# Aleph-Alpha/magma

Measured on NVIDIA H100. Metric: image-caption samples/sec (fwd+bwd), higher is better.
Workload: dtype bf16

## Files before the change

### magma_b200/csrc/attention.cu

```cuda
#include <stdlib.h>

#include "gemm_common.cuh"

namespace mb200 {

static constexpr int kAttThreads = 256;
static constexpr int kTile = 128 * 64 * 2;

struct AttnParams {
  int S, H, hd, rot;
  float scale;
  bf16* P;
  long long ldP;
  bf16* O;
  long long ldo;
  bf16* dqkv;
  long long ld_dqkv;
  const float2* rope_tab;
};

__device__ __forceinline__ void fence_async_smem() { asm volatile("fence.proxy.async.shared::cta;" ::: "memory"); }
__device__ __forceinline__ void wg_sync(int wg) { asm volatile("bar.sync %0, 128;" ::"r"(wg + 1) : "memory"); }

__device__ __forceinline__ uint32_t operand_off(int r, int c) {
  return (uint32_t)((c >> 6) * kTile + r * 128 + ((((c & 63) >> 3) ^ (r & 7)) << 4) + (c & 7) * 2);
}
__device__ __forceinline__ void st_pair(uint32_t saddr, float a, float b) {
  asm volatile("st.shared.b32 [%0], %1;" ::"r"(saddr), "r"(f32x2_to_bf16(a, b)) : "memory");
}
__device__ __forceinline__ float2 ld_pair(uint32_t saddr) {
  uint32_t u;
  asm volatile("ld.shared.b32 %0, [%1];" : "=r"(u) : "r"(saddr));
  return bf16x2_to_f32(u);
}
__device__ __forceinline__ float quad_max(float v) {
  v = fmaxf(v, __shfl_xor_sync(0xffffffffu, v, 1));
  return fmaxf(v, __shfl_xor_sync(0xffffffffu, v, 2));
}
__device__ __forceinline__ float quad_sum(float v) {
  v += __shfl_xor_sync(0xffffffffu, v, 1);
  return v + __shfl_xor_sync(0xffffffffu, v, 2);
}

template <int N, bool A_MN, bool B_MN>
__device__ __forceinline__ void wg_mma(float (&d)[N / 2], int wg, uint32_t a_base, uint32_t b_base, int nkb,
                                       uint32_t acc0 = 0u) {
  a_base += A_MN ? (uint32_t)(wg * kTile) : (uint32_t)(wg * 64 * 128);
  wgmma_fence();
  for (int kb = 0; kb < nkb; ++kb) {
#pragma unroll
    for (int k = 0; k < 4; ++k) {
      const uint32_t ao = A_MN ? (uint32_t)((kb * 4 + k) * 2048) : (uint32_t)(kb * kTile + k * 32);
      const uint32_t bo = B_MN ? (uint32_t)((kb * 4 + k) * 2048) : (uint32_t)(kb * kTile + k * 32);
      const uint64_t da = make_smem_desc(a_base + ao, A_MN ? (uint32_t)kTile : 0u, 1024);
      const uint64_t db = make_smem_desc(b_base + bo, B_MN ? (uint32_t)kTile : 0u, 1024);
      wgmma_bf16<N, A_MN ? 1 : 0, B_MN ? 1 : 0>(d, da, db, ((kb | k) != 0 ? 1u : 0u) | acc0);
    }
  }
  wgmma_commit();
  wgmma_wait<0>();
}

struct Frag {
  int wg, r0, c0, quad0;
  __device__ __forceinline__ Frag() {
    const int t = threadIdx.x;
    wg = t >> 7;
    r0 = wg * 64 + ((t & 127) >> 5) * 16 + ((t & 31) >> 2);
    c0 = 2 * (t & 3);
    quad0 = (t & 3) == 0;
  }
};

template <int HD>
__device__ __forceinline__ void store_rows(const Frag& f, const float (&d)[HD / 2], bf16* dst, long long ld, int nrows,
                                           const float2* tab, int rot) {
#pragma unroll
  for (int h = 0; h < 2; ++h) {
    const int r = f.r0 + 8 * h;
    if (r >= nrows) continue;
    bf16* row = dst + (long long)r * ld;
#pragma unroll
    for (int j = 0; j < HD / 8; ++j) {
      const int c = 8 * j + f.c0;
      float a0 = d[4 * j + 2 * h], a1 = d[4 * j + 2 * h + 1];
      if (tab != nullptr && c < rot) {
        const float2 cs = __ldg(tab + (long long)r * (rot >> 1) + (c >> 1));
        const float b0 = a0 * cs.x + a1 * cs.y;
        a1 = a1 * cs.x - a0 * cs.y;
        a0 = b0;
      }
      *reinterpret_cast<uint32_t*>(row + c) = f32x2_to_bf16(a0, a1);
    }
  }
}

template <int HD>
__global__ void __launch_bounds__(kAttThreads, 1)
attn_fwd_tile_kernel(const __grid_constant__ CUtensorMap tmQ, const __grid_constant__ CUtensorMap tmK,
                     const __grid_constant__ CUtensorMap tmV, const AttnParams p) {
  extern __shared__ uint8_t smem_raw[];
  uint8_t* smem = reinterpret_cast<uint8_t*>((reinterpret_cast<uintptr_t>(smem_raw) + 1023) & ~uintptr_t(1023));
  constexpr int nhb = HD / 64;
  uint8_t* sQ = smem;
  uint8_t* sK = sQ + nhb * kTile;
  uint8_t* sV = sK + nhb * kTile;
  uint8_t* sP = sV + nhb * kTile;
  uint64_t* bars = reinterpret_cast<uint64_t*>(sP + 2 * kTile);
  uint64_t* bar_qk = bars + 0;
  uint64_t* bar_v = bars + 1;

  const int t = threadIdx.x;
  const int h = blockIdx.x % p.H, b = blockIdx.x / p.H;
  const Frag f;

  pdl_trigger();
  if (t == 0) {
    tma_prefetch_desc(&tmQ);
    tma_prefetch_desc(&tmK);
    tma_prefetch_desc(&tmV);
    for (int i = 0; i < 2; ++i) mbar_init(&bars[i], 1);
    mbar_fence_init();
  }
  __syncthreads();
  pdl_wait();

  if (t == 0) {
    mbar_expect_tx(bar_qk, 2 * nhb * kTile);
    for (int kb = 0; kb < nhb; ++kb) {
      tma_load_4d(sQ + kb * kTile, &tmQ, bar_qk, kb * 64, 0, h, b);
      tma_load_4d(sK + kb * kTile, &tmK, bar_qk, kb * 64, 0, h, b);
    }
    mbar_expect_tx(bar_v, nhb * kTile);
    for (int kb = 0; kb < nhb; ++kb) tma_load_4d(sV + kb * kTile, &tmV, bar_v, kb * 64, 0, h, b);
  }
  mbar_wait(bar_qk, 0);
  float s[64];
  wg_mma<128, false, false>(s, f.wg, smem_u32(sQ), smem_u32(sK), nhb);
  const uint32_t sP_s = smem_u32(sP);
#pragma unroll
  for (int hh = 0; hh < 2; ++hh) {
    const int q = f.r0 + 8 * hh;
    const int lim = min(p.S, q + 1);
    float m = -INFINITY;
#pragma unroll
    for (int j = 0; j < 16; ++j)
#pragma unroll
      for (int e = 0; e < 2; ++e) {
        float& v = s[4 * j + 2 * hh + e];
        v *= p.scale;
        if (8 * j + f.c0 + e < lim) m = fmaxf(m, v);
      }
    m = quad_max(m);
    float sum = 0.f;
#pragma unroll
    for (int j = 0; j < 16; ++j)
#pragma unroll
      for (int e = 0; e < 2; ++e) {
        float& v = s[4 * j + 2 * hh + e];
        v = 8 * j + f.c0 + e < lim ? __expf(v - m) : 0.f;
        sum += v;
      }
    sum = quad_sum(sum);
    const float inv = q < p.S ? 1.f / sum : 0.f;
    bf16* prow = p.P + (((long long)b * p.H + h) * p.S + q) * p.ldP;
#pragma unroll
    for (int j = 0; j < 16; ++j) {
      const int c = 8 * j + f.c0;
      const float a0 = s[4 * j + 2 * hh] * inv, a1 = s[4 * j + 2 * hh + 1] * inv;
      st_pair(sP_s + operand_off(q, c), a0, a1);
      if (q < p.S && c < p.ldP) *reinterpret_cast<uint32_t*>(prow + c) = f32x2_to_bf16(a0, a1);
    }
  }
  fence_async_smem();
  wg_sync(f.wg);
  mbar_wait(bar_v, 0);
  float o[HD / 2];
  wg_mma<HD, false, true>(o, f.wg, sP_s, smem_u32(sV), 2);
// ... 121 lines not shown
  uint64_t* bars = reinterpret_cast<uint64_t*>(sP + 2 * kTile);
  uint64_t* bar_q = bars + 0;
  uint64_t* bar_k = bars + 1;
  uint64_t* bar_v = bars + 3;

  const int t = threadIdx.x;
  const int q0 = blockIdx.x * 128, h = blockIdx.y, b = blockIdx.z;
  const Frag f;

  pdl_trigger();
  if (t == 0) {
    tma_prefetch_desc(&tmQ);
    tma_prefetch_desc(&tmK);
    tma_prefetch_desc(&tmV);
    for (int i = 0; i < 5; ++i) mbar_init(&bars[i], 1);
    mbar_fence_init();
  }
  __syncthreads();
  pdl_wait();

  int n_kv = (p.Sk + 127) >> 7;
  if (p.causal) {
    const int last_key = min(p.Sk - 1, q0 + 127 + p.kv_off);
    n_kv = last_key < 0 ? 0 : min(n_kv, (last_key >> 7) + 1);
  }
  int row_lim[2];
  bool row_ok[2];
#pragma unroll
  for (int hh = 0; hh < 2; ++hh) {
    const int qi = q0 + f.r0 + 8 * hh;
    row_lim[hh] = !p.causal ? p.Sk : min(p.Sk, qi + p.kv_off + 1);
    row_ok[hh] = qi < p.Sq;
  }

  uint32_t ph_k[2] = {0, 0}, ph_v[2] = {0, 0};
  auto load_k = [&](int j, int buf) {
    mbar_expect_tx(&bar_k[buf], nhb * kTile);
    for (int kb = 0; kb < nhb; ++kb) tma_load_4d(sK + (buf * nhb + kb) * kTile, &tmK, &bar_k[buf], kb * 64, j * 128, h, b);
  };
  auto load_v = [&](int j, int buf) {
    mbar_expect_tx(&bar_v[buf], nhb * kTile);
    for (int kb = 0; kb < nhb; ++kb) tma_load_4d(sV + (buf * nhb + kb) * kTile, &tmV, &bar_v[buf], kb * 64, j * 128, h, b);
  };

  float m[2] = {-INFINITY, -INFINITY}, l[2] = {0.f, 0.f};
  if (t == 0 && n_kv > 0) {
    mbar_expect_tx(bar_q, nhb * kTile);
    for (int kb = 0; kb < nhb; ++kb) tma_load_4d(sQ + kb * kTile, &tmQ, bar_q, kb * 64, q0, h, b);
    load_k(0, 0);
  }
  if (n_kv > 0) mbar_wait(bar_q, 0);
  float s[64];
  for (int j = 0; j < n_kv; ++j) {
    const int buf = NBUF == 2 ? (j & 1) : 0;
    if (t == 0) {
      if (NBUF == 2 && j + 1 < n_kv) load_k(j + 1, (j + 1) & 1);
      if (NBUF == 1 && j + 1 < n_kv)
        for (int kb = 0; kb < nhb; ++kb) tma_prefetch_4d(&tmK, kb * 64, (j + 1) * 128, h, b);
    }
    mbar_wait(&bar_k[buf], ph_k[buf]);
    ph_k[buf] ^= 1;
    wg_mma<128, false, false>(s, f.wg, smem_u32(sQ), smem_u32(sK + buf * nhb * kTile), nhb);
    __syncthreads();
    if (NBUF == 1 && t == 0 && j + 1 < n_kv) load_k(j + 1, 0);
    const int kbase = j * 128;
#pragma unroll
    for (int hh = 0; hh < 2; ++hh) {
      float cm = -INFINITY;
#pragma unroll
      for (int jj = 0; jj < 16; ++jj)
#pragma unroll
        for (int e = 0; e < 2; ++e)
          if (kbase + 8 * jj + f.c0 + e < row_lim[hh]) cm = fmaxf(cm, s[4 * jj + 2 * hh + e] * p.scale);
      cm = quad_max(cm);
      if (cm > m[hh]) {
        l[hh] *= __expf(m[hh] - cm);
        m[hh] = cm;
      }
      if (m[hh] != -INFINITY) {
        float ls = 0.f;
#pragma unroll
        for (int jj = 0; jj < 16; ++jj)
#pragma unroll
          for (int e = 0; e < 2; ++e)
            if (kbase + 8 * jj + f.c0 + e < row_lim[hh]) ls += __expf(s[4 * jj + 2 * hh + e] * p.scale - m[hh]);
        l[hh] += quad_sum(ls);
      }
    }
  }
  float inv[2];
#pragma unroll
  for (int hh = 0; hh < 2; ++hh) {
    inv[hh] = (row_ok[hh] && l[hh] > 0.f) ? 1.f / l[hh] : 0.f;
    if (m[hh] == -INFINITY) m[hh] = 0.f;
    if (p.stats != nullptr && row_ok[hh] && f.quad0)
      p.stats[((long long)b * p.H + h) * p.Sq + q0 + f.r0 + 8 * hh] = make_float2(m[hh], inv[hh]);
  }

  const uint32_t sP_s = smem_u32(sP);
  if (t == 0 && n_kv > 0) {
    load_k(0, 0);
    load_v(0, 0);
  }
  float o[HD / 2];
#pragma unroll
  for (int i = 0; i < HD / 2; ++i) o[i] = 0.f;
  for (int j = 0; j < n_kv; ++j) {
    const int buf = NBUF == 2 ? (j & 1) : 0;
    if (t == 0) {
      if (NBUF == 2 && j + 1 < n_kv) {
        load_k(j + 1, (j + 1) & 1);
        load_v(j + 1, (j + 1) & 1);
      }
      if (NBUF == 1 && j + 1 < n_kv)
        for (int kb = 0; kb < nhb; ++kb) {
          tma_prefetch_4d(&tmK, kb * 64, (j + 1) * 128, h, b);
          tma_prefetch_4d(&tmV, kb * 64, (j + 1) * 128, h, b);
        }
    }
    mbar_wait(&bar_k[buf], ph_k[buf]);
    ph_k[buf] ^= 1;
    wg_mma<128, false, false>(s, f.wg, smem_u32(sQ), smem_u32(sK + buf * nhb * kTile), nhb);
    __syncthreads();
    if (NBUF == 1 && t == 0 && j + 1 < n_kv) load_k(j + 1, 0);
    const int kbase = j * 128;
#pragma unroll
    for (int hh = 0; hh < 2; ++hh) {
      const int r = f.r0 + 8 * hh;
      bf16* prow = p.P ? p.P + (((long long)b * p.H + h) * p.Sq + q0 + r) * p.ldP : nullptr;
#pragma unroll
      for (int jj = 0; jj < 16; ++jj) {
        const int c = 8 * jj + f.c0;
        float a[2];
#pragma unroll
        for (int e = 0; e < 2; ++e)
          a[e] = kbase + c + e < row_lim[hh] ? __expf(s[4 * jj + 2 * hh + e] * p.scale - m[hh]) * inv[hh] : 0.f;
        st_pair(sP_s + operand_off(r, c), a[0], a[1]);
        if (prow != nullptr && row_ok[hh] && kbase + c < p.ldP)
          *reinterpret_cast<uint32_t*>(prow + kbase + c) = f32x2_to_bf16(a[0], a[1]);
      }
    }
    fence_async_smem();
    wg_sync(f.wg);
    mbar_wait(&bar_v[buf], ph_v[buf]);
    ph_v[buf] ^= 1;
    wg_mma<HD, false, true>(o, f.wg, sP_s, smem_u32(sV + buf * nhb * kTile), 2, 1u);
    __syncthreads();
    if (NBUF == 1 && t == 0 && j + 1 < n_kv) load_v(j + 1, 0);
  }
  store_rows<HD>(f, o, p.O + ((long long)b * p.Sq + q0) * p.ldo + (long long)h * HD, p.ldo, p.Sq - q0, nullptr, 0);
  if (p.P != nullptr && t < 128 && q0 + t < p.Sq) {
    bf16* prow = p.P + (((long long)b * p.H + h) * p.Sq + q0 + t) * p.ldP;
    for (int col = n_kv * 128; col < p.ldP; col += 8) *reinterpret_cast<uint4*>(prow + col) = make_uint4(0, 0, 0, 0);
  }
}

static int tile_map(CUtensorMap* m, const void* ptr, long long ld, long long bs0, long long bs1, int rows, int cols,
                    int H, int B) {
  mb200_operand op;
  op.ptr = ptr;
  op.ld = ld;
  op.bs0 = bs0;
  op.bs1 = bs1;
  op.mn_major = 0;
  op.static_data = 0;
  return make_operand_map(m, op, rows, cols, H, B, 128);
}

static constexpr int smem_max = 232448;

bool attn_tile_supported(int S, int hd) { return S >= 1 && S <= 128 && hd >= 64 && hd <= 256 && hd % 64 == 0; }

int attn_fwd_tile(const bf16* qkv, long long ld_qkv, bf16* P, long long ldP, bf16* O, long long ldo, int B, int S, int H,
                  int hd, cudaStream_t st) {
  MB_REQUIRE(attn_tile_supported(S, hd) && ldP % 8 == 0, MB200_E_SHAPE, "attn_fwd_tile: unsupported S=%d hd=%d", S, hd);
  CUtensorMap tq, tk, tv;
  const long long d = (long long)H * hd;
  int rc;
  if ((rc = tile_map(&tq, qkv, ld_qkv, hd, (long long)S * ld_qkv, S, hd, H, B))) return rc;
  if ((rc = tile_map(&tk, qkv + d, ld_qkv, hd, (long long)S * ld_qkv, S, hd, H, B))) return rc;
  if ((rc = tile_map(&tv, qkv + 2 * d, ld_qkv, hd, (long long)S * ld_qkv, S, hd, H, B))) return rc;
  AttnParams p;
  memset(&p, 0, sizeof(p));
  p.S = S;
  p.H = H;
  p.hd = hd;
  p.scale = 1.0f / sqrtf((float)hd);
  p.P = P;
  p.ldP = ldP;
  p.O = O;
  p.ldo = ldo;
  const int smem = (3 * (hd / 64) + 2) * kTile + 1024 + 128;
#define MB_FWD(HD)                                                                                                   \
  {                                                                                                                  \
    static bool set = false;                                                                                         \
    if (!set) {                                                                                                      \
      MB_CUDA(cudaFuncSetAttribute(attn_fwd_tile_kernel<HD>, cudaFuncAttributeMaxDynamicSharedMemorySize, smem_max)); \
      set = true;                                                                                                    \
    }                                                                                                                \
    MB_CUDA(launch_pdl(attn_fwd_tile_kernel<HD>, dim3(B * H), dim3(kAttThreads), (size_t)smem, st, tq, tk, tv, p));  \
  }
  switch (hd) {
    case 64: MB_FWD(64) break;
    case 128: MB_FWD(128) break;
    case 192: MB_FWD(192) break;
    default: MB_FWD(256) break;
  }
#undef MB_FWD
  count_launch();
  return 0;
}

int attn_bwd_tile(const bf16* qkv, long long ld_qkv, const bf16* dO, long long ld_do, const bf16* P, long long ldP,
                  bf16* dqkv, long long ld_dqkv, const float* rope_tab, int rot, int B, int S, int H, int hd,
                  cudaStream_t st) {
  MB_REQUIRE(attn_tile_supported(S, hd) && ldP % 8 == 0, MB200_E_SHAPE, "attn_bwd_tile: unsupported S=%d hd=%d", S, hd);
  CUtensorMap tq, tk, tv, tdo, tp;
  const long long d = (long long)H * hd;
  int rc;
  if ((rc = tile_map(&tq, qkv, ld_qkv, hd, (long long)S * ld_qkv, S, hd, H, B))) return rc;
  if ((rc = tile_map(&tk, qkv + d, ld_qkv, hd, (long long)S * ld_qkv, S, hd, H, B))) return rc;
  if ((rc = tile_map(&tv, qkv + 2 * d, ld_qkv, hd, (long long)S * ld_qkv, S, hd, H, B))) return rc;
  if ((rc = tile_map(&tdo, dO, ld_do, hd, (long long)S * ld_do, S, hd, H, B))) return rc;
  if ((rc = tile_map(&tp, P, ldP, (long long)S * ldP, (long long)H * S * ldP, S, S, H, B))) return rc;
  AttnParams p;
  memset(&p, 0, sizeof(p));
  p.S = S;
  p.H = H;
  p.hd = hd;
  p.rot = rot;
  p.scale = 1.0f / sqrtf((float)hd);
  p.P = const_cast<bf16*>(P);
  p.ldP = ldP;
  p.dqkv = dqkv;
  p.ld_dqkv = ld_dqkv;
  p.rope_tab = reinterpret_cast<const float2*>(rope_tab);
  const int smem = (2 * (hd / 64) + 4) * kTile + 1024 + 128;
#define MB_BWD(HD)                                                                                                   \
  {                                                                                                                  \
    static bool set = false;                                                                                         \
    if (!set) {                                                                                                      \
      MB_CUDA(cudaFuncSetAttribute(attn_bwd_tile_kernel<HD>, cudaFuncAttributeMaxDynamicSharedMemorySize, smem_max)); \
      set = true;                                                                                                    \
    }                                                                                                                \
    MB_CUDA(launch_pdl(attn_bwd_tile_kernel<HD>, dim3(B * H), dim3(kAttThreads), (size_t)smem, st, tq, tk, tv, tdo,  \
                       tp, p));                                                                                      \
  }
  switch (hd) {
    case 64: MB_BWD(64) break;
    case 128: MB_BWD(128) break;
    case 192: MB_BWD(192) break;
    default: MB_BWD(256) break;
  }
#undef MB_BWD
  count_launch();
  return 0;
}

bool attn_flash_supported(int hd) { return hd >= 64 && hd <= 256 && hd % 64 == 0; }

int attn_fwd_flash(const bf16* q, long long ldq, long long q_bsh, long long q_bsb, const bf16* k, long long ldk,
                   long long k_bsh, long long k_bsb, const bf16* v, long long ldv, long long v_bsh, long long v_bsb,
                   bf16* O, long long ldo, bf16* P, long long ldP, float* stats, int B, int Sq, int Sk, int H, int hd,
                   int causal, cudaStream_t st) {
  MB_REQUIRE(attn_flash_supported(hd) && Sq >= 1 && Sk >= 1 && B >= 1 && H >= 1, MB200_E_SHAPE,
             "attn_fwd_flash: unsupported Sq=%d Sk=%d hd=%d", Sq, Sk, hd);
  MB_REQUIRE(!causal || Sk >= Sq, MB200_E_SHAPE, "attn_fwd_flash: causal needs Sk >= Sq (%d < %d)", Sk, Sq);
  MB_REQUIRE(P == nullptr || (ldP % 8 == 0 && ldP >= Sk), MB200_E_ALIGN, "attn_fwd_flash: ldP=%lld must be >= Sk and %%8",
             ldP);
  MB_REQUIRE(ldo % 8 == 0 && (reinterpret_cast<uintptr_t>(O) & 15) == 0, MB200_E_ALIGN, "attn_fwd_flash: O alignment");
  CUtensorMap tq, tk, tv;
  int rc;
  if ((rc = tile_map(&tq, q, ldq, q_bsh, q_bsb, Sq, hd, H, B))) return rc;
  if ((rc = tile_map(&tk, k, ldk, k_bsh, k_bsb, Sk, hd, H, B))) return rc;
  if ((rc = tile_map(&tv, v, ldv, v_bsh, v_bsb, Sk, hd, H, B))) return rc;
  FlashParams p;
  memset(&p, 0, sizeof(p));
  p.Sq = Sq;
  p.Sk = Sk;
  p.H = H;
  p.hd = hd;
  p.causal = causal;
  p.kv_off = Sk - Sq;
  p.scale = 1.0f / sqrtf((float)hd);
  p.O = O;
  p.ldo = ldo;
  p.P = P;
  p.ldP = ldP;
  p.stats = reinterpret_cast<float2*>(stats);
  const dim3 grid((Sq + 127) / 128, H, B);
#define MB_FLASH(HD, NB)                                                                                             \
  {                                                                                                                  \
    const int smem = ((1 + 2 * NB) * (HD / 64) + 2) * kTile + 1024 + 128;                                           \
    static bool set = false;                                                                                         \
    if (!set) {                                                                                                      \
      MB_CUDA(cudaFuncSetAttribute(attn_fwd_flash_kernel<HD, NB>, cudaFuncAttributeMaxDynamicSharedMemorySize,      \
                                   smem_max));                                                                       \
      set = true;                                                                                                    \
    }                                                                                                                \
    MB_CUDA(launch_pdl(attn_fwd_flash_kernel<HD, NB>, grid, dim3(kAttThreads), (size_t)smem, st, tq, tk, tv, p));    \
  }
  switch (hd) {
    case 64: MB_FLASH(64, 2) break;
    case 128: MB_FLASH(128, 2) break;
    case 192: MB_FLASH(192, 1) break;
    default: MB_FLASH(256, 1) break;
  }
#undef MB_FLASH
  count_launch();
  return 0;
}

}

extern "C" int mb200_attn_fwd_tile(const void* qkv, int64_t ld_qkv, void* P, int64_t ldP, void* O, int64_t ldo, int32_t B,
                                   int32_t S, int32_t H, int32_t hd, void* stream) {
  int rc = mb200::check_arch();
  if (rc) return rc;
  return mb200::attn_fwd_tile((const mb200::bf16*)qkv, ld_qkv, (mb200::bf16*)P, ldP, (mb200::bf16*)O, ldo, B, S, H, hd,
                              (cudaStream_t)stream);
}

extern "C" int mb200_attn_bwd_tile(const void* qkv, int64_t ld_qkv, const void* dO, int64_t ld_do, const void* P,
                                   int64_t ldP, void* dqkv, int64_t ld_dqkv, const float* rope_tab, int32_t rot,
                                   int32_t B, int32_t S, int32_t H, int32_t hd, void* stream) {
  int rc = mb200::check_arch();
  if (rc) return rc;
  return mb200::attn_bwd_tile((const mb200::bf16*)qkv, ld_qkv, (const mb200::bf16*)dO, ld_do, (const mb200::bf16*)P, ldP,
                              (mb200::bf16*)dqkv, ld_dqkv, rope_tab, rot, B, S, H, hd, (cudaStream_t)stream);
}

extern "C" int mb200_attn_fwd_flash(const void* q, int64_t ldq, int64_t q_bsh, int64_t q_bsb, const void* k, int64_t ldk,
                                    int64_t k_bsh, int64_t k_bsb, const void* v, int64_t ldv, int64_t v_bsh, int64_t v_bsb,
                                    void* O, int64_t ldo, void* P, int64_t ldP, float* stats, int32_t B, int32_t Sq,
                                    int32_t Sk, int32_t H, int32_t hd, int32_t causal, void* stream) {
  int rc = mb200::check_arch();
  if (rc) return rc;
  return mb200::attn_fwd_flash((const mb200::bf16*)q, ldq, q_bsh, q_bsb, (const mb200::bf16*)k, ldk, k_bsh, k_bsb,
                               (const mb200::bf16*)v, ldv, v_bsh, v_bsb, (mb200::bf16*)O, ldo, (mb200::bf16*)P, ldP, stats,
                               B, Sq, Sk, H, hd, causal, (cudaStream_t)stream);
}
```

### magma_b200/csrc/wgmma.cuh

```cuda

__device__ __forceinline__ void wgmma_fence() { asm volatile("wgmma.fence.sync.aligned;" ::: "memory"); }
__device__ __forceinline__ void wgmma_commit() { asm volatile("wgmma.commit_group.sync.aligned;" ::: "memory"); }
template <int N>
__device__ __forceinline__ void wgmma_wait() { asm volatile("wgmma.wait_group.sync.aligned %0;" ::"n"(N) : "memory"); }

__device__ __forceinline__ uint64_t make_smem_desc(uint32_t saddr, uint32_t lbo_bytes, uint32_t sbo_bytes) {
  uint64_t d = 0;
  d |= (uint64_t)((saddr >> 4) & 0x3FFF);
  d |= (uint64_t)((lbo_bytes >> 4) & 0x3FFF) << 16;
  d |= (uint64_t)((sbo_bytes >> 4) & 0x3FFF) << 32;
  d |= (uint64_t)1 << 62;
  return d;
}

template <int TA, int TB>
__device__ __forceinline__ void wgmma_bf16_n64(float (&d)[32], uint64_t da, uint64_t db, uint32_t accumulate) {
  asm volatile(
      "{\n\t"
      ".reg .pred p;\n\t"
      "setp.ne.b32 p, %34, 0;\n\t"
      "wgmma.mma_async.sync.aligned.m64n64k16.f32.bf16.bf16 "
      "{%0, %1, %2, %3, %4, %5, %6, %7, %8, %9, %10, %11, %12, %13, %14, %15, %16, %17, %18, %19, %20, %21, %22, %23, %24, %25, %26, %27, %28, %29, %30, %31}, "
      "%32, %33, p, 1, 1, %35, %36;\n\t"
      "}\n"
      : "+f"(d[0]), "+f"(d[1]), "+f"(d[2]), "+f"(d[3]), "+f"(d[4]), "+f"(d[5]), "+f"(d[6]), "+f"(d[7]), "+f"(d[8]), "+f"(d[9]), "+f"(d[10]), "+f"(d[11]), "+f"(d[12]), "+f"(d[13]), "+f"(d[14]), "+f"(d[15]), "+f"(d[16]), "+f"(d[17]), "+f"(d[18]), "+f"(d[19]), "+f"(d[20]), "+f"(d[21]), "+f"(d[22]), "+f"(d[23]), "+f"(d[24]), "+f"(d[25]), "+f"(d[26]), "+f"(d[27]), "+f"(d[28]), "+f"(d[29]), "+f"(d[30]), "+f"(d[31])
      : "l"(da), "l"(db), "r"(accumulate), "n"(TA), "n"(TB));
}

template <int TA, int TB>
__device__ __forceinline__ void wgmma_bf16_n128(float (&d)[64], uint64_t da, uint64_t db, uint32_t accumulate) {
  asm volatile(
      "{\n\t"
      ".reg .pred p;\n\t"
      "setp.ne.b32 p, %66, 0;\n\t"
      "wgmma.mma_async.sync.aligned.m64n128k16.f32.bf16.bf16 "
      "{%0, %1, %2, %3, %4, %5, %6, %7, %8, %9, %10, %11, %12, %13, %14, %15, %16, %17, %18, %19, %20, %21, %22, %23, %24, %25, %26, %27, %28, %29, %30, %31, %32, %33, %34, %35, %36, %37, %38, %39, %40, %41, %42, %43, %44, %45, %46, %47, %48, %49, %50, %51, %52, %53, %54, %55, %56, %57, %58, %59, %60, %61, %62, %63}, "
      "%64, %65, p, 1, 1, %67, %68;\n\t"
      "}\n"
      : "+f"(d[0]), "+f"(d[1]), "+f"(d[2]), "+f"(d[3]), "+f"(d[4]), "+f"(d[5]), "+f"(d[6]), "+f"(d[7]), "+f"(d[8]), "+f"(d[9]), "+f"(d[10]), "+f"(d[11]), "+f"(d[12]), "+f"(d[13]), "+f"(d[14]), "+f"(d[15]), "+f"(d[16]), "+f"(d[17]), "+f"(d[18]), "+f"(d[19]), "+f"(d[20]), "+f"(d[21]), "+f"(d[22]), "+f"(d[23]), "+f"(d[24]), "+f"(d[25]), "+f"(d[26]), "+f"(d[27]), "+f"(d[28]), "+f"(d[29]), "+f"(d[30]), "+f"(d[31]), "+f"(d[32]), "+f"(d[33]), "+f"(d[34]), "+f"(d[35]), "+f"(d[36]), "+f"(d[37]), "+f"(d[38]), "+f"(d[39]), "+f"(d[40]), "+f"(d[41]), "+f"(d[42]), "+f"(d[43]), "+f"(d[44]), "+f"(d[45]), "+f"(d[46]), "+f"(d[47]), "+f"(d[48]), "+f"(d[49]), "+f"(d[50]), "+f"(d[51]), "+f"(d[52]), "+f"(d[53]), "+f"(d[54]), "+f"(d[55]), "+f"(d[56]), "+f"(d[57]), "+f"(d[58]), "+f"(d[59]), "+f"(d[60]), "+f"(d[61]), "+f"(d[62]), "+f"(d[63])
      : "l"(da), "l"(db), "r"(accumulate), "n"(TA), "n"(TB));
}

template <int TA, int TB>
__device__ __forceinline__ void wgmma_bf16_n192(float (&d)[96], uint64_t da, uint64_t db, uint32_t accumulate) {
  asm volatile(
      "{\n\t"
      ".reg .pred p;\n\t"
      "setp.ne.b32 p, %98, 0;\n\t"
      "wgmma.mma_async.sync.aligned.m64n192k16.f32.bf16.bf16 "
      "{%0, %1, %2, %3, %4, %5, %6, %7, %8, %9, %10, %11, %12, %13, %14, %15, %16, %17, %18, %19, %20, %21, %22, %23, %24, %25, %26, %27, %28, %29, %30, %31, %32, %33, %34, %35, %36, %37, %38, %39, %40, %41, %42, %43, %44, %45, %46, %47, %48, %49, %50, %51, %52, %53, %54, %55, %56, %57, %58, %59, %60, %61, %62, %63, %64, %65, %66, %67, %68, %69, %70, %71, %72, %73, %74, %75, %76, %77, %78, %79, %80, %81, %82, %83, %84, %85, %86, %87, %88, %89, %90, %91, %92, %93, %94, %95}, "
      "%96, %97, p, 1, 1, %99, %100;\n\t"
      "}\n"
      : "+f"(d[0]), "+f"(d[1]), "+f"(d[2]), "+f"(d[3]), "+f"(d[4]), "+f"(d[5]), "+f"(d[6]), "+f"(d[7]), "+f"(d[8]), "+f"(d[9]), "+f"(d[10]), "+f"(d[11]), "+f"(d[12]), "+f"(d[13]), "+f"(d[14]), "+f"(d[15]), "+f"(d[16]), "+f"(d[17]), "+f"(d[18]), "+f"(d[19]), "+f"(d[20]), "+f"(d[21]), "+f"(d[22]), "+f"(d[23]), "+f"(d[24]), "+f"(d[25]), "+f"(d[26]), "+f"(d[27]), "+f"(d[28]), "+f"(d[29]), "+f"(d[30]), "+f"(d[31]), "+f"(d[32]), "+f"(d[33]), "+f"(d[34]), "+f"(d[35]), "+f"(d[36]), "+f"(d[37]), "+f"(d[38]), "+f"(d[39]), "+f"(d[40]), "+f"(d[41]), "+f"(d[42]), "+f"(d[43]), "+f"(d[44]), "+f"(d[45]), "+f"(d[46]), "+f"(d[47]), "+f"(d[48]), "+f"(d[49]), "+f"(d[50]), "+f"(d[51]), "+f"(d[52]), "+f"(d[53]), "+f"(d[54]), "+f"(d[55]), "+f"(d[56]), "+f"(d[57]), "+f"(d[58]), "+f"(d[59]), "+f"(d[60]), "+f"(d[61]), "+f"(d[62]), "+f"(d[63]), "+f"(d[64]), "+f"(d[65]), "+f"(d[66]), "+f"(d[67]), "+f"(d[68]), "+f"(d[69]), "+f"(d[70]), "+f"(d[71]), "+f"(d[72]), "+f"(d[73]), "+f"(d[74]), "+f"(d[75]), "+f"(d[76]), "+f"(d[77]), "+f"(d[78]), "+f"(d[79]), "+f"(d[80]), "+f"(d[81]), "+f"(d[82]), "+f"(d[83]), "+f"(d[84]), "+f"(d[85]), "+f"(d[86]), "+f"(d[87]), "+f"(d[88]), "+f"(d[89]), "+f"(d[90]), "+f"(d[91]), "+f"(d[92]), "+f"(d[93]), "+f"(d[94]), "+f"(d[95])
      : "l"(da), "l"(db), "r"(accumulate), "n"(TA), "n"(TB));
}

template <int TA, int TB>
__device__ __forceinline__ void wgmma_bf16_n256(float (&d)[128], uint64_t da, uint64_t db, uint32_t accumulate) {
  asm volatile(
      "{\n\t"
      ".reg .pred p;\n\t"
      "setp.ne.b32 p, %130, 0;\n\t"
      "wgmma.mma_async.sync.aligned.m64n256k16.f32.bf16.bf16 "
      "{%0, %1, %2, %3, %4, %5, %6, %7, %8, %9, %10, %11, %12, %13, %14, %15, %16, %17, %18, %19, %20, %21, %22, %23, %24, %25, %26, %27, %28, %29, %30, %31, %32, %33, %34, %35, %36, %37, %38, %39, %40, %41, %42, %43, %44, %45, %46, %47, %48, %49, %50, %51, %52, %53, %54, %55, %56, %57, %58, %59, %60, %61, %62, %63, %64, %65, %66, %67, %68, %69, %70, %71, %72, %73, %74, %75, %76, %77, %78, %79, %80, %81, %82, %83, %84, %85, %86, %87, %88, %89, %90, %91, %92, %93, %94, %95, %96, %97, %98, %99, %100, %101, %102, %103, %104, %105, %106, %107, %108, %109, %110, %111, %112, %113, %114, %115, %116, %117, %118, %119, %120, %121, %122, %123, %124, %125, %126, %127}, "
      "%128, %129, p, 1, 1, %131, %132;\n\t"
      "}\n"
      : "+f"(d[0]), "+f"(d[1]), "+f"(d[2]), "+f"(d[3]), "+f"(d[4]), "+f"(d[5]), "+f"(d[6]), "+f"(d[7]), "+f"(d[8]), "+f"(d[9]), "+f"(d[10]), "+f"(d[11]), "+f"(d[12]), "+f"(d[13]), "+f"(d[14]), "+f"(d[15]), "+f"(d[16]), "+f"(d[17]), "+f"(d[18]), "+f"(d[19]), "+f"(d[20]), "+f"(d[21]), "+f"(d[22]), "+f"(d[23]), "+f"(d[24]), "+f"(d[25]), "+f"(d[26]), "+f"(d[27]), "+f"(d[28]), "+f"(d[29]), "+f"(d[30]), "+f"(d[31]), "+f"(d[32]), "+f"(d[33]), "+f"(d[34]), "+f"(d[35]), "+f"(d[36]), "+f"(d[37]), "+f"(d[38]), "+f"(d[39]), "+f"(d[40]), "+f"(d[41]), "+f"(d[42]), "+f"(d[43]), "+f"(d[44]), "+f"(d[45]), "+f"(d[46]), "+f"(d[47]), "+f"(d[48]), "+f"(d[49]), "+f"(d[50]), "+f"(d[51]), "+f"(d[52]), "+f"(d[53]), "+f"(d[54]), "+f"(d[55]), "+f"(d[56]), "+f"(d[57]), "+f"(d[58]), "+f"(d[59]), "+f"(d[60]), "+f"(d[61]), "+f"(d[62]), "+f"(d[63]), "+f"(d[64]), "+f"(d[65]), "+f"(d[66]), "+f"(d[67]), "+f"(d[68]), "+f"(d[69]), "+f"(d[70]), "+f"(d[71]), "+f"(d[72]), "+f"(d[73]), "+f"(d[74]), "+f"(d[75]), "+f"(d[76]), "+f"(d[77]), "+f"(d[78]), "+f"(d[79]), "+f"(d[80]), "+f"(d[81]), "+f"(d[82]), "+f"(d[83]), "+f"(d[84]), "+f"(d[85]), "+f"(d[86]), "+f"(d[87]), "+f"(d[88]), "+f"(d[89]), "+f"(d[90]), "+f"(d[91]), "+f"(d[92]), "+f"(d[93]), "+f"(d[94]), "+f"(d[95]), "+f"(d[96]), "+f"(d[97]), "+f"(d[98]), "+f"(d[99]), "+f"(d[100]), "+f"(d[101]), "+f"(d[102]), "+f"(d[103]), "+f"(d[104]), "+f"(d[105]), "+f"(d[106]), "+f"(d[107]), "+f"(d[108]), "+f"(d[109]), "+f"(d[110]), "+f"(d[111]), "+f"(d[112]), "+f"(d[113]), "+f"(d[114]), "+f"(d[115]), "+f"(d[116]), "+f"(d[117]), "+f"(d[118]), "+f"(d[119]), "+f"(d[120]), "+f"(d[121]), "+f"(d[122]), "+f"(d[123]), "+f"(d[124]), "+f"(d[125]), "+f"(d[126]), "+f"(d[127])
      : "l"(da), "l"(db), "r"(accumulate), "n"(TA), "n"(TB));
}

template <int N, int TA, int TB>
__device__ __forceinline__ void wgmma_bf16(float (&d)[N / 2], uint64_t da, uint64_t db, uint32_t accumulate) {
  static_assert(N == 64 || N == 128 || N == 192 || N == 256, "wgmma_bf16: N must be 64, 128, 192 or 256");
  if constexpr (N == 64) wgmma_bf16_n64<TA, TB>(d, da, db, accumulate);
  else if constexpr (N == 128) wgmma_bf16_n128<TA, TB>(d, da, db, accumulate);
  else if constexpr (N == 192) wgmma_bf16_n192<TA, TB>(d, da, db, accumulate);
  else wgmma_bf16_n256<TA, TB>(d, da, db, accumulate);
}
```

Measured before the change: 158.8.

## Add specialized short-key flash attention forward kernel for head dim 64

Adds a dedicated forward attention kernel for non-causal hd=64 with up to 272 keys. It loads all of K and V once per block in 64-row TMA boxes, computes scores with one m64n256 plus one m64n16 wgmma per k-step, and does the whole softmax in one pass with no online rescaling across KV tiles. Each CTA handles up to five 64-row query slabs split across two warpgroups, which cuts per-tile loop overhead and barriers. The cost is a large register footprint (128+8 score floats per thread) and a hard-coded key limit.

```diff
diff --git a/magma_b200/csrc/attention.cu b/magma_b200/csrc/attention.cu
--- a/magma_b200/csrc/attention.cu
+++ b/magma_b200/csrc/attention.cu
@@ -22,8 +22,8 @@
 __device__ __forceinline__ void fence_async_smem() { asm volatile("fence.proxy.async.shared::cta;" ::: "memory"); }
 __device__ __forceinline__ void wg_sync(int wg) { asm volatile("bar.sync %0, 128;" ::"r"(wg + 1) : "memory"); }
 
-__device__ __forceinline__ uint32_t operand_off(int r, int c) {
-  return (uint32_t)((c >> 6) * kTile + r * 128 + ((((c & 63) >> 3) ^ (r & 7)) << 4) + (c & 7) * 2);
+__device__ __forceinline__ uint32_t operand_off(int r, int c, uint32_t kb_bytes = kTile) {
+  return (uint32_t)((c >> 6) * kb_bytes + r * 128 + ((((c & 63) >> 3) ^ (r & 7)) << 4) + (c & 7) * 2);
 }
 __device__ __forceinline__ void st_pair(uint32_t saddr, float a, float b) {
   asm volatile("st.shared.b32 [%0], %1;" ::"r"(saddr), "r"(f32x2_to_bf16(a, b)) : "memory");
@@ -454,8 +454,152 @@
   }
 }
 
+static constexpr int kShortKeys = 272;
+static constexpr int kShortBlocks = 5;
+static constexpr int kBox64 = 64 * 64 * 2;
+
+__global__ void __launch_bounds__(kAttThreads, 1)
+attn_fwd_shortkey_kernel(const __grid_constant__ CUtensorMap tmQ, const __grid_constant__ CUtensorMap tmK,
+                         const __grid_constant__ CUtensorMap tmV, const FlashParams p) {
+  extern __shared__ uint8_t smem_raw[];
+  uint8_t* smem = reinterpret_cast<uint8_t*>((reinterpret_cast<uintptr_t>(smem_raw) + 1023) & ~uintptr_t(1023));
+  uint8_t* sQ = smem;
+  uint8_t* sK = sQ + kShortBlocks * kBox64;
+  uint8_t* sV = sK + kShortBlocks * kBox64;
+  uint8_t* sP = sV + kShortBlocks * kBox64;
+  uint64_t* bars = reinterpret_cast<uint64_t*>(sP + 2 * kShortBlocks * kBox64);
+  uint64_t* bar_qk = bars + 0;
+  uint64_t* bar_v = bars + 1;
+
+  const int t = threadIdx.x;
+  const int q0 = blockIdx.x * kShortBlocks * 64, h = blockIdx.y, b = blockIdx.z;
+  const int nslab = min(kShortBlocks, (p.Sq - q0 + 63) >> 6);
+  const int nkb = (p.Sk + 63) >> 6;
+  const Frag f;
+  const int lr0 = f.r0 & 63;
+
+  pdl_trigger();
+  if (t == 0) {
+    tma_prefetch_desc(&tmQ);
+    tma_prefetch_desc(&tmK);
+    tma_prefetch_desc(&tmV);
+    for (int i = 0; i < 2; ++i) mbar_init(&bars[i], 1);
+    mbar_fence_init();
+  }
+  for (int kb = nkb; kb < kShortBlocks; ++kb) {
+    for (int i = t; i < kBox64 / 16; i += kAttThreads) {
+      reinterpret_cast<uint4*>(sK + kb * kBox64)[i] = make_uint4(0, 0, 0, 0);
+      reinterpret_cast<uint4*>(sV + kb * kBox64)[i] = make_uint4(0, 0, 0, 0);
+    }
+  }
+  fence_async_smem();
+  __syncthreads();
+  pdl_wait();
+
+  if (t == 0) {
+    mbar_expect_tx(bar_qk, (nslab + nkb) * kBox64);
+    for (int s = 0; s < nslab; ++s) tma_load_4d(sQ + s * kBox64, &tmQ, bar_qk, 0, q0 + s * 64, h, b);
+    for (int kb = 0; kb < nkb; ++kb) tma_load_4d(sK + kb * kBox64, &tmK, bar_qk, 0, kb * 64, h, b);
+    mbar_expect_tx(bar_v, nkb * kBox64);
+    for (int kb = 0; kb < nkb; ++kb) tma_load_4d(sV + kb * kBox64, &tmV, bar_v, 0, kb * 64, h, b);
+  }
+  const uint32_t sP_s = smem_u32(sP) + (uint32_t)(f.wg * kShortBlocks * kBox64);
+  const uint32_t sK_s = smem_u32(sK), sV_s = smem_u32(sV);
+  mbar_wait(bar_qk, 0);
+  bool v_ready = false;
+  for (int slab = f.wg; slab < nslab; slab += 2) {
+    const int qs = q0 + slab * 64;
+    float s0[128], s1[8];
+    {
+      const uint32_t a = smem_u32(sQ) + (uint32_t)(slab * kBox64);
+      wgmma_fence();
+#pragma unroll
+      for (int k = 0; k < 4; ++k) {
+        const uint64_t da = make_smem_desc(a + k * 32, 0u, 1024);
+        wgmma_bf16<256, 0, 0>(s0, da, make_smem_desc(sK_s + k * 32, 0u, 1024), k != 0 ? 1u : 0u);
+        wgmma_bf16<16, 0, 0>(s1, da, make_smem_desc(sK_s + 4 * kBox64 + k * 32, 0u, 1024), k != 0 ? 1u : 0u);
+      }
+      wgmma_commit();
+      wgmma_wait<0>();
+    }
+#pragma unroll
+    for (int hh = 0; hh < 2; ++hh) {
+      const int lr = lr0 + 8 * hh, q = qs + lr;
+      const bool row_ok = q < p.Sq;
+      float m = -INFINITY, l = 0.f;
+#pragma unroll
+      for (int ch = 0; ch < 3; ++ch) {
+        const int j0 = ch < 2 ? 16 * ch : 0, nj = ch < 2 ? 16 : 2;
+        float* sc = ch < 2 ? s0 : s1;
+        float cm = -INFINITY;
+#pragma unroll
+        for (int jj = 0; jj < nj; ++jj)
+#pragma unroll
+          for (int e = 0; e < 2; ++e)
+            cm = fmaxf(cm, 128 * ch + 8 * jj + f.c0 + e < p.Sk ? sc[4 * (j0 + jj) + 2 * hh + e] * p.scale : -INFINITY);
+        cm = quad_max(cm);
+        if (cm > m) {
+          l *= __expf(m - cm);
+          m = cm;
+        }
+        if (m != -INFINITY) {
+          float ls = 0.f;
+#pragma unroll
+          for (int jj = 0; jj < nj; ++jj)
+#pragma unroll
+            for (int e = 0; e < 2; ++e)
+              ls += 128 * ch + 8 * jj + f.c0 + e < p.Sk ? __expf(sc[4 * (j0 + jj) + 2 * hh + e] * p.scale - m) : 0.f;
+          l += quad_sum(ls);
+        }
+      }
+      const float inv = 1.f / l;
+      if (p.stats != nullptr && row_ok && f.quad0)
+        p.stats[((long long)b * p.H + h) * p.Sq + q] = make_float2(m, inv);
+      bf16* prow = p.P != nullptr && row_ok ? p.P + (((long long)b * p.H + h) * p.Sq + q) * p.ldP : nullptr;
+#pragma unroll
+      for (int j = 0; j < kShortBlocks * 8; ++j) {
+        const int c = 8 * j + f.c0;
+        float a[2];
+#pragma unroll
+        for (int e = 0; e < 2; ++e) {
+          const float sv = j < 32 ? s0[4 * j + 2 * hh + e] : j < 34 ? s1[4 * (j - 32) + 2 * hh + e] : 0.f;
+          a[e] = c + e < p.Sk ? __expf(sv * p.scale - m) * inv : 0.f;
+        }
+        const float a0 = a[0], a1 = a[1];
+        st_pair(sP_s + operand_off(lr, c, kBox64), a0, a1);
+        if (prow != nullptr && c < p.ldP) *reinterpret_cast<uint32_t*>(prow + c) = f32x2_to_bf16(a0, a1);
+      }
+      if (prow != nullptr)
+        for (int c = 64 * kShortBlocks + f.c0; c < p.ldP; c += 8) *reinterpret_cast<uint32_t*>(prow + c) = 0u;
+    }
+    fence_async_smem();
+    wg_sync(f.wg);
+    if (!v_ready) {
+      mbar_wait(bar_v, 0);
+      v_ready = true;
+    }
+    float o[32];
+    wgmma_fence();
+#pragma unroll
+    for (int kb = 0; kb < kShortBlocks; ++kb) {
+#pragma unroll
+      for (int k = 0; k < 4; ++k) {
+        const uint64_t da = make_smem_desc(sP_s + kb * kBox64 + k * 32, 0u, 1024);
+        const uint64_t db = make_smem_desc(sV_s + (kb * 4 + k) * 2048, (uint32_t)kTile, 1024);
+        wgmma_bf16<64, 0, 1>(o, da, db, (kb | k) != 0 ? 1u : 0u);
+      }
+    }
+    wgmma_commit();
+    wgmma_wait<0>();
+    Frag fs = f;
+    fs.r0 = lr0;
+    store_rows<64>(fs, o, p.O + ((long long)b * p.Sq + qs) * p.ldo + (long long)h * 64, p.ldo, p.Sq - qs, nullptr, 0);
+    wg_sync(f.wg);
+  }
+}
+
 static int tile_map(CUtensorMap* m, const void* ptr, long long ld, long long bs0, long long bs1, int rows, int cols,
-                    int H, int B) {
+                    int H, int B, int box_rows = 128) {
   mb200_operand op;
   op.ptr = ptr;
   op.ld = ld;
@@ -463,7 +607,7 @@
   op.bs1 = bs1;
   op.mn_major = 0;
   op.static_data = 0;
-  return make_operand_map(m, op, rows, cols, H, B, 128);
+  return make_operand_map(m, op, rows, cols, H, B, box_rows);
 }
 
 static constexpr int smem_max = 232448;
@@ -568,11 +712,13 @@
   MB_REQUIRE(P == nullptr || (ldP % 8 == 0 && ldP >= Sk), MB200_E_ALIGN, "attn_fwd_flash: ldP=%lld must be >= Sk and %%8",
              ldP);
   MB_REQUIRE(ldo % 8 == 0 && (reinterpret_cast<uintptr_t>(O) & 15) == 0, MB200_E_ALIGN, "attn_fwd_flash: O alignment");
+  const bool short_keys = !causal && hd == 64 && Sk <= kShortKeys;
+  const int box = short_keys ? 64 : 128;
   CUtensorMap tq, tk, tv;
   int rc;
-  if ((rc = tile_map(&tq, q, ldq, q_bsh, q_bsb, Sq, hd, H, B))) return rc;
-  if ((rc = tile_map(&tk, k, ldk, k_bsh, k_bsb, Sk, hd, H, B))) return rc;
-  if ((rc = tile_map(&tv, v, ldv, v_bsh, v_bsb, Sk, hd, H, B))) return rc;
+  if ((rc = tile_map(&tq, q, ldq, q_bsh, q_bsb, Sq, hd, H, B, box))) return rc;
+  if ((rc = tile_map(&tk, k, ldk, k_bsh, k_bsb, Sk, hd, H, B, box))) return rc;
+  if ((rc = tile_map(&tv, v, ldv, v_bsh, v_bsb, Sk, hd, H, B, box))) return rc;
   FlashParams p;
   memset(&p, 0, sizeof(p));
   p.Sq = Sq;
@@ -587,6 +733,18 @@
   p.P = P;
   p.ldP = ldP;
   p.stats = reinterpret_cast<float2*>(stats);
+  if (short_keys) {
+    const int smem = 5 * kShortBlocks * kBox64 + 1024 + 128;
+    static bool set = false;
+    if (!set) {
+      MB_CUDA(cudaFuncSetAttribute(attn_fwd_shortkey_kernel, cudaFuncAttributeMaxDynamicSharedMemorySize, smem_max));
+      set = true;
+    }
+    const dim3 grid((Sq + 64 * kShortBlocks - 1) / (64 * kShortBlocks), H, B);
+    MB_CUDA(launch_pdl(attn_fwd_shortkey_kernel, grid, dim3(kAttThreads), (size_t)smem, st, tq, tk, tv, p));
+    count_launch();
+    return 0;
+  }
   const dim3 grid((Sq + 127) / 128, H, B);
 #define MB_FLASH(HD, NB)                                                                                             \
   {                                                                                                                  \
diff --git a/magma_b200/csrc/wgmma.cuh b/magma_b200/csrc/wgmma.cuh
--- a/magma_b200/csrc/wgmma.cuh
+++ b/magma_b200/csrc/wgmma.cuh
@@ -11,6 +11,20 @@
   d |= (uint64_t)((sbo_bytes >> 4) & 0x3FFF) << 32;
   d |= (uint64_t)1 << 62;
   return d;
+}
+
+template <int TA, int TB>
+__device__ __forceinline__ void wgmma_bf16_n16(float (&d)[8], uint64_t da, uint64_t db, uint32_t accumulate) {
+  asm volatile(
+      "{\n\t"
+      ".reg .pred p;\n\t"
+      "setp.ne.b32 p, %10, 0;\n\t"
+      "wgmma.mma_async.sync.aligned.m64n16k16.f32.bf16.bf16 "
+      "{%0, %1, %2, %3, %4, %5, %6, %7}, "
+      "%8, %9, p, 1, 1, %11, %12;\n\t"
+      "}\n"
+      : "+f"(d[0]), "+f"(d[1]), "+f"(d[2]), "+f"(d[3]), "+f"(d[4]), "+f"(d[5]), "+f"(d[6]), "+f"(d[7])
+      : "l"(da), "l"(db), "r"(accumulate), "n"(TA), "n"(TB));
 }
 
 template <int TA, int TB>
@@ -71,8 +85,9 @@
 
 template <int N, int TA, int TB>
 __device__ __forceinline__ void wgmma_bf16(float (&d)[N / 2], uint64_t da, uint64_t db, uint32_t accumulate) {
-  static_assert(N == 64 || N == 128 || N == 192 || N == 256, "wgmma_bf16: N must be 64, 128, 192 or 256");
-  if constexpr (N == 64) wgmma_bf16_n64<TA, TB>(d, da, db, accumulate);
+  static_assert(N == 16 || N == 64 || N == 128 || N == 192 || N == 256, "wgmma_bf16: N must be 16, 64, 128, 192 or 256");
+  if constexpr (N == 16) wgmma_bf16_n16<TA, TB>(d, da, db, accumulate);
+  else if constexpr (N == 64) wgmma_bf16_n64<TA, TB>(d, da, db, accumulate);
   else if constexpr (N == 128) wgmma_bf16_n128<TA, TB>(d, da, db, accumulate);
   else if constexpr (N == 192) wgmma_bf16_n192<TA, TB>(d, da, db, accumulate);
   else wgmma_bf16_n256<TA, TB>(d, da, db, accumulate);
```

After: 160.9, median of 6. 1.3% higher.

## Add single-pass attention forward kernel for hd64 with short key length

Applied to the files above, without the earlier changes.

Adds a specialized forward attention kernel for head dim 64 and key length up to 272. It loads all K/V tiles into shared memory at once, computes the full score row in one pass with an exact softmax, and processes three query tiles per CTA so each K/V load is reused across them. A new m64n16 wgmma variant covers the 16-column tail. This removes the online-softmax rescaling and the per-tile K/V streaming, at the cost of high register and shared-memory use and a narrow shape-specific code path.

```diff
diff --git a/magma_b200/csrc/attention.cu b/magma_b200/csrc/attention.cu
--- a/magma_b200/csrc/attention.cu
+++ b/magma_b200/csrc/attention.cu
@@ -451,6 +451,165 @@
   if (p.P != nullptr && t < 128 && q0 + t < p.Sq) {
     bf16* prow = p.P + (((long long)b * p.H + h) * p.Sq + q0 + t) * p.ldP;
     for (int col = n_kv * 128; col < p.ldP; col += 8) *reinterpret_cast<uint4*>(prow + col) = make_uint4(0, 0, 0, 0);
+  }
+}
+
+static constexpr int kOnepassMaxSk = 272, kOnepassQTiles = 3;
+
+__global__ void __launch_bounds__(kAttThreads, 1)
+attn_fwd_onepass_kernel(const __grid_constant__ CUtensorMap tmQ, const __grid_constant__ CUtensorMap tmK,
+                        const __grid_constant__ CUtensorMap tmV, const FlashParams p) {
+  extern __shared__ uint8_t smem_raw[];
+  uint8_t* smem = reinterpret_cast<uint8_t*>((reinterpret_cast<uintptr_t>(smem_raw) + 1023) & ~uintptr_t(1023));
+  uint8_t* sQ = smem;
+  uint8_t* sK = sQ + kOnepassQTiles * kTile;
+  uint8_t* sV = sK + 3 * kTile;
+  uint8_t* sP = sV + 3 * kTile;
+  uint64_t* bars = reinterpret_cast<uint64_t*>(sP + 5 * kTile);
+  uint64_t* bar_qk = bars + 0;
+  uint64_t* bar_v = bars + 1;
+
+  const int t = threadIdx.x;
+  const int qt0 = blockIdx.x * kOnepassQTiles, h = blockIdx.y, b = blockIdx.z;
+  const int n_qt = min(kOnepassQTiles, (p.Sq + 127) / 128 - qt0);
+  const int n_kt = (p.Sk + 127) >> 7;
+  const Frag f;
+
+  pdl_trigger();
+  if (t == 0) {
+    tma_prefetch_desc(&tmQ);
+    tma_prefetch_desc(&tmK);
+    tma_prefetch_desc(&tmV);
+    for (int i = 0; i < 2; ++i) mbar_init(&bars[i], 1);
+    mbar_fence_init();
+  }
+  __syncthreads();
+  pdl_wait();
+
+  if (t == 0) {
+    mbar_expect_tx(bar_qk, (n_qt + n_kt) * kTile);
+    for (int i = 0; i < n_qt; ++i) tma_load_4d(sQ + i * kTile, &tmQ, bar_qk, 0, (qt0 + i) * 128, h, b);
+    for (int j = 0; j < n_kt; ++j) tma_load_4d(sK + j * kTile, &tmK, bar_qk, 0, j * 128, h, b);
+    mbar_expect_tx(bar_v, n_kt * kTile);
+    for (int j = 0; j < n_kt; ++j) tma_load_4d(sV + j * kTile, &tmV, bar_v, 0, j * 128, h, b);
+  }
+  mbar_wait(bar_qk, 0);
+  const uint32_t sK_s = smem_u32(sK), sV_s = smem_u32(sV), sP_s = smem_u32(sP);
+  const uint32_t sPa = sP_s + (uint32_t)(f.wg * 64 * 128);
+  const int n_ks = (p.Sk + 15) >> 4;
+
+  for (int i = 0; i < n_qt; ++i) {
+    const int q0 = (qt0 + i) * 128;
+    if (q0 + f.wg * 64 >= p.Sq) break;
+    float s0[64], s1[64], s2[8];
+    const uint32_t qa = smem_u32(sQ + i * kTile) + (uint32_t)(f.wg * 64 * 128);
+    wgmma_fence();
+#pragma unroll
+    for (int k = 0; k < 4; ++k) {
+      const uint64_t da = make_smem_desc(qa + k * 32, 0, 1024);
+      const uint32_t acc = k != 0 ? 1u : 0u;
+      wgmma_bf16<128, 0, 0>(s0, da, make_smem_desc(sK_s + k * 32, 0, 1024), acc);
+      if (p.Sk > 128) wgmma_bf16<128, 0, 0>(s1, da, make_smem_desc(sK_s + kTile + k * 32, 0, 1024), acc);
+      if (p.Sk > 256) wgmma_bf16<16, 0, 0>(s2, da, make_smem_desc(sK_s + 2 * kTile + k * 32, 0, 1024), acc);
+    }
+    wgmma_commit();
+    wgmma_wait<0>();
+#pragma unroll
+    for (int hh = 0; hh < 2; ++hh) {
+      const int r = f.r0 + 8 * hh, qi = q0 + r;
+      const bool ok = qi < p.Sq;
+      const int lim = !p.causal ? p.Sk : min(p.Sk, qi + p.kv_off + 1);
+      float cm0 = -INFINITY, cm1 = -INFINITY, cm2 = -INFINITY;
+#pragma unroll
+      for (int jj = 0; jj < 16; ++jj)
+#pragma unroll
+        for (int e = 0; e < 2; ++e) {
+          const int c = 8 * jj + f.c0 + e;
+          if (c < lim) cm0 = fmaxf(cm0, __fmul_rn(s0[4 * jj + 2 * hh + e], p.scale));
+          if (c + 128 < lim) cm1 = fmaxf(cm1, __fmul_rn(s1[4 * jj + 2 * hh + e], p.scale));
+          if (jj < 2 && c + 256 < lim) cm2 = fmaxf(cm2, __fmul_rn(s2[4 * jj + 2 * hh + e], p.scale));
+        }
+      cm0 = quad_max(cm0);
+      cm1 = quad_max(cm1);
+      cm2 = quad_max(cm2);
+      const float m0 = cm0, m1 = fmaxf(m0, cm1), m = fmaxf(m1, cm2);
+      float ls0 = 0.f, ls1 = 0.f, ls2 = 0.f;
+      const bool re0 = __any_sync(0xffffffffu, m0 != m), re1 = __any_sync(0xffffffffu, m1 != m);
+      if (re0)
+#pragma unroll
+        for (int jj = 0; jj < 16; ++jj)
+#pragma unroll
+          for (int e = 0; e < 2; ++e)
+            if (8 * jj + f.c0 + e < lim) ls0 += __expf(__fmaf_rn(s0[4 * jj + 2 * hh + e], p.scale, -m0));
+      if (re1)
+#pragma unroll
+        for (int jj = 0; jj < 16; ++jj)
+#pragma unroll
+          for (int e = 0; e < 2; ++e)
+            if (128 + 8 * jj + f.c0 + e < lim) ls1 += __expf(__fmaf_rn(s1[4 * jj + 2 * hh + e], p.scale, -m1));
+#pragma unroll
+      for (int jj = 0; jj < 16; ++jj)
+#pragma unroll
+        for (int e = 0; e < 2; ++e) {
+          const int c = 8 * jj + f.c0 + e;
+          float& v0 = s0[4 * jj + 2 * hh + e];
+          float& v1 = s1[4 * jj + 2 * hh + e];
+          v0 = c < lim ? __expf(__fmaf_rn(v0, p.scale, -m)) : 0.f;
+          v1 = c + 128 < lim ? __expf(__fmaf_rn(v1, p.scale, -m)) : 0.f;
+          if (!re0) ls0 += v0;
+          if (!re1) ls1 += v1;
+          if (jj < 2) {
+            float& v2 = s2[4 * jj + 2 * hh + e];
+            v2 = c + 256 < lim ? __expf(__fmaf_rn(v2, p.scale, -m)) : 0.f;
+            ls2 += v2;
+          }
+        }
+      ls0 = quad_sum(ls0);
+      ls1 = quad_sum(ls1);
+      ls2 = quad_sum(ls2);
+      float l = 0.f, mr = -INFINITY;
+      const float cms[3] = {cm0, cm1, cm2}, lss[3] = {ls0, ls1, ls2};
+#pragma unroll
+      for (int g = 0; g < 3; ++g) {
+        if (g * 128 >= p.Sk) break;
+        if (cms[g] > mr) {
+          l *= __expf(mr - cms[g]);
+          mr = cms[g];
+        }
+        if (mr != -INFINITY) l += lss[g];
+      }
+      const float inv = ok && l > 0.f ? 1.f / l : 0.f;
+      if (p.stats != nullptr && ok && f.quad0) p.stats[((long long)b * p.H + h) * p.Sq + qi] = make_float2(m, inv);
+      bf16* prow = p.P != nullptr && ok ? p.P + (((long long)b * p.H + h) * p.Sq + qi) * p.ldP : nullptr;
+      auto put = [&](int c, float a0, float a1) {
+        st_pair(sP_s + operand_off(r, c), a0, a1);
+        if (prow != nullptr && c < p.ldP) *reinterpret_cast<uint32_t*>(prow + c) = f32x2_to_bf16(a0, a1);
+      };
+#pragma unroll
+      for (int jj = 0; jj < 16; ++jj) {
+        const int c = 8 * jj + f.c0;
+        put(c, s0[4 * jj + 2 * hh] * inv, s0[4 * jj + 2 * hh + 1] * inv);
+        put(c + 128, s1[4 * jj + 2 * hh] * inv, s1[4 * jj + 2 * hh + 1] * inv);
+        if (jj < 2) put(c + 256, s2[4 * jj + 2 * hh] * inv, s2[4 * jj + 2 * hh + 1] * inv);
+      }
+      if (prow != nullptr)
+        for (int col = kOnepassMaxSk + 8 * (t & 3); col < p.ldP; col += 32)
+          *reinterpret_cast<uint4*>(prow + col) = make_uint4(0, 0, 0, 0);
+    }
+    fence_async_smem();
+    wg_sync(f.wg);
+    mbar_wait(bar_v, 0);
+    float o[32];
+    wgmma_fence();
+    for (int ks = 0; ks < n_ks; ++ks) {
+      const uint64_t da = make_smem_desc(sPa + (ks >> 2) * kTile + (ks & 3) * 32, 0, 1024);
+      const uint64_t db = make_smem_desc(sV_s + ks * 2048, kTile, 1024);
+      wgmma_bf16<64, 0, 1>(o, da, db, ks != 0 ? 1u : 0u);
+    }
+    wgmma_commit();
+    wgmma_wait<0>();
+    store_rows<64>(f, o, p.O + ((long long)b * p.Sq + q0) * p.ldo + (long long)h * 64, p.ldo, p.Sq - q0, nullptr, 0);
+    wg_sync(f.wg);
   }
 }
 
@@ -587,6 +746,18 @@
   p.P = P;
   p.ldP = ldP;
   p.stats = reinterpret_cast<float2*>(stats);
+  if (hd == 64 && Sk <= kOnepassMaxSk) {
+    const int smem = (kOnepassQTiles + 3 + 3 + 5) * kTile + 1024 + 128;
+    static bool set = false;
+    if (!set) {
+      MB_CUDA(cudaFuncSetAttribute(attn_fwd_onepass_kernel, cudaFuncAttributeMaxDynamicSharedMemorySize, smem_max));
+      set = true;
+    }
+    const dim3 grid(((Sq + 127) / 128 + kOnepassQTiles - 1) / kOnepassQTiles, H, B);
+    MB_CUDA(launch_pdl(attn_fwd_onepass_kernel, grid, dim3(kAttThreads), (size_t)smem, st, tq, tk, tv, p));
+    count_launch();
+    return 0;
+  }
   const dim3 grid((Sq + 127) / 128, H, B);
 #define MB_FLASH(HD, NB)                                                                                             \
   {                                                                                                                  \
diff --git a/magma_b200/csrc/wgmma.cuh b/magma_b200/csrc/wgmma.cuh
--- a/magma_b200/csrc/wgmma.cuh
+++ b/magma_b200/csrc/wgmma.cuh
@@ -11,6 +11,20 @@
   d |= (uint64_t)((sbo_bytes >> 4) & 0x3FFF) << 32;
   d |= (uint64_t)1 << 62;
   return d;
+}
+
+template <int TA, int TB>
+__device__ __forceinline__ void wgmma_bf16_n16(float (&d)[8], uint64_t da, uint64_t db, uint32_t accumulate) {
+  asm volatile(
+      "{\n\t"
+      ".reg .pred p;\n\t"
+      "setp.ne.b32 p, %10, 0;\n\t"
+      "wgmma.mma_async.sync.aligned.m64n16k16.f32.bf16.bf16 "
+      "{%0, %1, %2, %3, %4, %5, %6, %7}, "
+      "%8, %9, p, 1, 1, %11, %12;\n\t"
+      "}\n"
+      : "+f"(d[0]), "+f"(d[1]), "+f"(d[2]), "+f"(d[3]), "+f"(d[4]), "+f"(d[5]), "+f"(d[6]), "+f"(d[7])
+      : "l"(da), "l"(db), "r"(accumulate), "n"(TA), "n"(TB));
 }
 
 template <int TA, int TB>
@@ -71,8 +85,10 @@
 
 template <int N, int TA, int TB>
 __device__ __forceinline__ void wgmma_bf16(float (&d)[N / 2], uint64_t da, uint64_t db, uint32_t accumulate) {
-  static_assert(N == 64 || N == 128 || N == 192 || N == 256, "wgmma_bf16: N must be 64, 128, 192 or 256");
-  if constexpr (N == 64) wgmma_bf16_n64<TA, TB>(d, da, db, accumulate);
+  static_assert(N == 16 || N == 64 || N == 128 || N == 192 || N == 256,
+                "wgmma_bf16: N must be 16, 64, 128, 192 or 256");
+  if constexpr (N == 16) wgmma_bf16_n16<TA, TB>(d, da, db, accumulate);
+  else if constexpr (N == 64) wgmma_bf16_n64<TA, TB>(d, da, db, accumulate);
   else if constexpr (N == 128) wgmma_bf16_n128<TA, TB>(d, da, db, accumulate);
   else if constexpr (N == 192) wgmma_bf16_n192<TA, TB>(d, da, db, accumulate);
   else wgmma_bf16_n256<TA, TB>(d, da, db, accumulate);
```

Result: faster. 161.1 before, 163.1 after, median of 6 (+1.2%).
